# KillingSpark/zstd-rs

Measured on AMD Instinct MI355X. Metric: decompressed_GB_per_s, higher is better.
Workload: dtype u8

## Files before the change

### zstd-rs_amd/csrc/zg_dev.h

```cpp
#pragma once
#include <stdint.h>
#include "zg_types.h"

#if defined(__HIPCC__)
#include <hip/hip_runtime.h>
#define ZG_HD __host__ __device__ __forceinline__
#else
#define ZG_HD static inline __attribute__((always_inline))
#endif

static constexpr uint32_t ZG_LL_BASE[36] = {0, 1, 2, 3, 4, 5, 6, 7, 8, 9, 10, 11, 12, 13, 14, 15, 16, 18, 20, 22, 24, 28, 32, 40,
                                            48, 64, 128, 256, 512, 1024, 2048, 4096, 8192, 16384, 32768, 65536};
static constexpr uint8_t ZG_LL_BITS[36] = {0, 0, 0, 0, 0, 0, 0, 0, 0, 0, 0, 0, 0, 0, 0, 0, 1, 1, 1, 1, 2, 2, 3, 3,
                                           4, 6, 7, 8, 9, 10, 11, 12, 13, 14, 15, 16};
static constexpr uint32_t ZG_ML_BASE[53] = {3, 4, 5, 6, 7, 8, 9, 10, 11, 12, 13, 14, 15, 16, 17, 18, 19, 20, 21, 22, 23, 24, 25, 26, 27, 28, 29,
                                            30, 31, 32, 33, 34, 35, 37, 39, 41, 43, 47, 51, 59, 67, 83, 99, 131, 259, 515, 1027, 2051, 4099,
                                            8195, 16387, 32771, 65539};
static constexpr uint8_t ZG_ML_BITS[53] = {0, 0, 0, 0, 0, 0, 0, 0, 0, 0, 0, 0, 0, 0, 0, 0, 0, 0, 0, 0, 0, 0, 0, 0, 0, 0, 0,
                                           0, 0, 0, 0, 0, 1, 1, 1, 1, 2, 2, 3, 3, 4, 4, 5, 7, 8, 9, 10, 11, 12, 13, 14, 15, 16};
static constexpr int16_t ZG_LL_DEFAULT[36] = {4, 3, 2, 2, 2, 2, 2, 2, 2, 2, 2, 2, 2, 1, 1, 1, 2, 2, 2, 2, 2, 2, 2, 2, 2, 3, 2, 1, 1, 1, 1, 1, -1, -1, -1, -1};
static constexpr int16_t ZG_ML_DEFAULT[53] = {1, 4, 3, 2, 2, 2, 2, 2, 2, 1, 1, 1, 1, 1, 1, 1, 1, 1, 1, 1, 1, 1, 1, 1, 1, 1, 1, 1, 1, 1, 1, 1,
                                              1, 1, 1, 1, 1, 1, 1, 1, 1, 1, 1, 1, 1, 1, -1, -1, -1, -1, -1, -1, -1};
static constexpr int16_t ZG_OF_DEFAULT[29] = {1, 1, 1, 1, 1, 1, 2, 2, 2, 1, 1, 1, 1, 1, 1, 1, 1, 1, 1, 1, 1, 1, 1, 1, -1, -1, -1, -1, -1};

// ... 115 lines not shown
        pos = (pos + step) & (size - 1);
        if (++guard > size) return ZG_INTERNAL;
      }
    }
  }
  if (placed != neg) return ZG_INTERNAL;
  for (uint32_t i = 0; i < neg; i++) {
    unsigned s = out[i];
    uint32_t p = (uint32_t)probs[s], k = counter[s]++;
    unsigned hb = zg_hbit(p);
    uint32_t slices = ((1u << (hb - 1)) == p) ? p : (1u << hb);
    uint32_t dbl = slices - p, single = p - dbl, width = size / slices;
    uint32_t nb = zg_hbit(width) - 1, bl;
    if (k < dbl) { bl = single * width + k * width * 2; nb += 1; }
    else bl = (k - dbl) * width;
    out[i] = zg_fse_pack(kind, bl, nb, s);
  }
  for (uint32_t i = neg; i < size; i++) out[i] = zg_fse_pack(kind, 0, (uint32_t)acc_log, out[i]);
  return ZG_OK;
}

ZG_HD int zg_huf_read_weights(const uint8_t* src, uint32_t len, uint8_t* weights, int* nweights, uint32_t* bytes_used, uint32_t* fse_tab,
                              int16_t* probs, uint16_t* counter) {
  if (len == 0) return ZG_HUF_TABLE;
  uint32_t header = src[0];
  uint32_t bits_read = 8;
  if (header < 128) {
    const uint8_t* fs = src + 1;
    uint32_t flen = len - 1;
    if (header > flen) return ZG_HUF_TABLE;
    int np, al;
    uint32_t used;
    int st = zg_fse_read_probs(fs, flen, 6, 255, probs, &np, &al, &used);
    if (st) return ZG_HUF_TABLE;
    st = zg_fse_build(probs, np, al, ZG_KIND_HUFW, fse_tab, counter);
    if (st) return st == ZG_INTERNAL ? st : ZG_HUF_TABLE;
    if (used > header) return ZG_HUF_TABLE;
    uint32_t clen = header - used;
    const uint8_t* cs = fs + used;
    bits_read += (used + clen) * 8;
    if (clen == 0) return ZG_HUF_TABLE;
    uint32_t lastb = cs[clen - 1];
    if (lastb == 0) return ZG_HUF_TABLE;
    int32_t P = (int32_t)(clen - 1) * 8 + (int32_t)(zg_hbit(lastb) - 1);
    uint32_t e1, e2;
    P -= al; e1 = fse_tab[zg_bits_at_z(cs, P, (unsigned)al)];
    P -= al; e2 = fse_tab[zg_bits_at_z(cs, P, (unsigned)al)];
    int n = 0;
    for (;;) {
      weights[n++] = (uint8_t)ZG_FSEW_SYM(e1);
      { unsigned nb = ZG_FSE_NB(e1); P -= nb; e1 = fse_tab[ZG_FSE_BL(e1) + zg_bits_at_z(cs, P, nb)]; }
      if (P <= -1) { weights[n++] = (uint8_t)ZG_FSEW_SYM(e2); break; }
      weights[n++] = (uint8_t)ZG_FSEW_SYM(e2);
      { unsigned nb = ZG_FSE_NB(e2); P -= nb; e2 = fse_tab[ZG_FSE_BL(e2) + zg_bits_at_z(cs, P, nb)]; }
      if (P <= -1) { weights[n++] = (uint8_t)ZG_FSEW_SYM(e1); break; }
      if (n > 255) return ZG_HUF_TABLE;
    }
    *nweights = n;
  } else {
    uint32_t n = header - 127, need = (n + 1) / 2;
    if (len - 1 < need) return ZG_HUF_TABLE;
    for (uint32_t i = 0; i < n; i++) {
      uint8_t b = src[1 + i / 2];
      weights[i] = (i & 1) ? (b & 0xF) : (b >> 4);
      bits_read += 4;
    }
    *nweights = (int)n;
  }
  *bytes_used = (bits_read + 7) >> 3;
  return ZG_OK;
}

ZG_HD int zg_huf_build(const uint8_t* weights, int nweights, uint16_t* out, int* max_bits_out) {
  uint32_t weight_sum = 0;
  for (int i = 0; i < nweights; i++) {
    unsigned w = weights[i];
    if (w > 11) return ZG_HUF_TABLE;
    weight_sum += w ? (1u << (w - 1)) : 0u;
  }
  if (weight_sum == 0) return ZG_HUF_TABLE;
  unsigned max_bits = zg_hbit(weight_sum);
  uint32_t left = (1u << max_bits) - weight_sum;
  if (left & (left - 1)) return ZG_HUF_TABLE;
  unsigned last_weight = zg_hbit(left);
  if (max_bits > 11) return ZG_HUF_TABLE;
  *max_bits_out = (int)max_bits;
  uint32_t rank_count[13];
  for (int i = 0; i < 13; i++) rank_count[i] = 0;
  for (int s = 0; s <= nweights; s++) {
    unsigned w = s < nweights ? weights[s] : last_weight;
    unsigned b = w ? max_bits + 1 - w : 0;
    rank_count[b]++;
  }
  uint32_t rank_idx[13];
  rank_idx[max_bits] = 0;
  for (unsigned b = max_bits; b >= 1; b--) rank_idx[b - 1] = rank_idx[b] + rank_count[b] * (1u << (max_bits - b));
  uint32_t size = 1u << max_bits;
  if (rank_idx[0] != size) return ZG_INTERNAL;
  for (int s = 0; s <= nweights; s++) {
    unsigned w = s < nweights ? weights[s] : last_weight;
    if (!w) continue;
    unsigned b = max_bits + 1 - w;
    uint32_t base = rank_idx[b], n = 1u << (max_bits - b);
    rank_idx[b] += n;
    uint16_t e = ZG_HUF_PACK((unsigned)(s & 255), b);
    for (uint32_t i = 0; i < n; i++) out[base + i] = e;
  }
  return ZG_OK;
}

#define ZG_OFF_HUGE 0x3FFFFFFFu
#define ZG_SYM_TAG(v) ((v) >> 30)
#define ZG_SYM_K(v) ((v) & 0x3FFFFFFFu)
ZG_HD uint32_t zg_sym_dec(uint32_t v) {
  const uint32_t c = v ? v - 1 : 0u;
  return ZG_SYM_TAG(v) ? v + 1 : c;
}
ZG_HD uint32_t zg_sym_resolve(uint32_t v, const uint32_t* h) {
  uint32_t t = ZG_SYM_TAG(v);
  if (!t) return v;
  const uint32_t x = t == 1 ? h[0] : t == 2 ? h[1] : h[2], k = ZG_SYM_K(v);
  return x > k ? x - k : 0;
}
ZG_HD uint32_t zg_hist_step(uint32_t of, uint32_t ll, uint32_t& h0, uint32_t& h1, uint32_t& h2) {
  const bool isnew = of > 3u;
  const uint32_t c = ll ? of : of + 1u;
  const uint32_t rep = c == 1u ? h0 : c == 2u ? h1 : c == 3u ? h2 : zg_sym_dec(h0);
  const uint32_t actual = isnew ? of - 3u : rep;
  const bool rot = isnew || c >= 3u;
  const bool moved = rot || c == 2u;
  h2 = rot ? h1 : h2;
  h1 = moved ? h0 : h1;
  h0 = actual;
  return actual;
}
struct ZgHistMap { uint32_t s[3]; };
ZG_HD ZgHistMap zg_map_identity() { return {{1u << 30, 2u << 30, 3u << 30}}; }
ZG_HD uint32_t zg_map_apply(const ZgHistMap& A, uint32_t v) {
  const uint32_t t = ZG_SYM_TAG(v);
  if (!t) return v;
  const uint32_t a = t == 1 ? A.s[0] : t == 2 ? A.s[1] : A.s[2], k = ZG_SYM_K(v);
  if (ZG_SYM_TAG(a)) {
    uint32_t kk = ZG_SYM_K(a) + k;
    if (kk > 0x3FFFFFFFu) kk = 0x3FFFFFFFu;
    return (a & 0xC0000000u) | kk;
  }
  return a > k ? a - k : 0;
}
ZG_HD ZgHistMap zg_map_compose(const ZgHistMap& A, const ZgHistMap& B) {
  ZgHistMap r;
  r.s[0] = zg_map_apply(A, B.s[0]); r.s[1] = zg_map_apply(A, B.s[1]); r.s[2] = zg_map_apply(A, B.s[2]);
  return r;
}
```

### zstd-rs_amd/csrc/zg_kernels.hip

```cpp
#include <stdlib.h>
#include "zg_kernels.h"
#include "zg_dev.h"
#include "zg_xxh64_dev.h"
#include "zg_scatter.h"

#define ZG_SEQ_G 16
#define ZG_LZ_T 256

typedef uint32_t zg_v4u __attribute__((ext_vector_type(4)));
typedef __attribute__((address_space(1))) zg_v4u zg_gv4u;
typedef uint32_t zg_v2u __attribute__((ext_vector_type(2)));
typedef __attribute__((address_space(1))) zg_v2u zg_gv2u;
typedef uint32_t zg_v3u __attribute__((ext_vector_type(3)));
typedef __attribute__((address_space(1))) zg_v3u zg_gv3u;
__device__ __forceinline__ uint32_t zg_ld32_fun(const uint8_t* p) {
  const uint64_t a = (uint64_t)p;
  const zg_v2u v = *(const zg_gv2u*)(a & ~3ull);
  return __builtin_amdgcn_alignbit(v.y, v.x, ((uint32_t)a & 3u) * 8u);
}

__device__ __forceinline__ void zg_set_status(uint32_t* status, uint32_t b, int st) {
  if (st) atomicCAS(&status[b], 0u, (uint32_t)st);
}
__device__ __forceinline__ uint32_t zg_sweep_window(const ZgBatchDev& d, const ZgFrame& fr) {
// ... 622 lines not shown
    if (!s_ok[g]) {
      const uint32_t bo = d.aux[b].seq_bits_off;
      const bool nopad = bo <= blk.src_len && (blk.src_len == bo || d.src[blk.src_off + blk.src_len - 1u] == 0);
      if (owner && !mover) zg_set_status(d.status, b, nopad ? ZG_SEQ_EXTRA_PADDING : ZG_FSE_UNINIT);
      act = false;
    } else {
      const uint32_t bits_off = d.aux[b].seq_bits_off;
      if (bits_off > blk.src_len) { if (owner && !mover) zg_set_status(d.status, b, ZG_INTERNAL); act = false; }
      else {
        const uint8_t* bs = d.src + blk.src_off + bits_off;
        const uint32_t bs_len = blk.src_len - bits_off;
        nseq = blk.nseq;
        const uint32_t lastb = bs_len ? bs[bs_len - 1] : 0;
        if (bs_len == 0 || lastb == 0) { if (owner && !mover) zg_set_status(d.status, b, ZG_SEQ_EXTRA_PADDING); act = false; }
        else {
          P = (int32_t)(bs_len - 1) * 8 + (int32_t)(zg_hbit(lastb) - 1);
          bsA = (uint64_t)bs;
          rbits = (int32_t)((uint32_t)(bsA & (ZG_SEQ_RING - 1)) * 8u);
          floorA = (bsA & ~15ull) - 16;
          dstp = (uint64_t)(d.raw_arena + blk.seq_base);
          have = true;
        }
      }
    }
  }
  {
    uint64_t top = 0, want = 0;
    if (act) {
      top = (bsA + (uint64_t)(P >> 3) + 8 + 15) & ~15ull;
      const uint64_t p0 = bsA + (uint64_t)(P >> 3);
      want = p0 > ZG_SEQ_MARGIN + 16 ? (p0 - ZG_SEQ_MARGIN - 16) & ~15ull : 0;
      if (want < floorA) want = floorA;
      lo = want;
    }
    if (owner && !mover) { s_fetch_hi[g] = act ? top : 0; s_fetch_lo[g] = act ? want : 0; }
    __syncthreads();
    for (uint32_t j = t; j < ZG_SEQ_G * ZG_SEQ_PRO; j += 128) {
      const uint32_t gg = j / ZG_SEQ_PRO, k = j % ZG_SEQ_PRO;
      const uint64_t hi = s_fetch_hi[gg], addr = hi - 16ull * (k + 1);
      if (hi && addr >= s_fetch_lo[gg] && addr < hi) { const zg_v4u v = *(const zg_gv4u*)addr; zg_ring_put(s_ring[gg], addr, v); }
    }
    __syncthreads();
  }
  ZgSeqChain c = {0, 0, 0, 0, 0, 0, 0, 0, 0};
  if (act) {
    const uint32_t ll_log = s_log[g][0], of_log = s_log[g][1], ml_log = s_log[g][2];
    const uint32_t lg = role == 0u ? of_log : role == 1u ? ml_log : role == 2u ? ll_log : 0u;
    const int32_t q = P - (int32_t)(role == 2u ? ll_log : role == 0u ? ll_log + of_log : ll_log + of_log + ml_log);
    c.st = (q >= 0 && role != 3u) ? zg_ring_bits(store, q + rbits, lg) : 0u;
    c.e = ZG_SEQ_LD16(tab, c.st); c.s = PK ? 0u : ZG_SEQ_LD8(xtab, c.st);
    P -= (int32_t)(ll_log + of_log + ml_log);
    if (owner && !mover) d.seq_out[b].pad = (uint32_t)P;
    left = nseq;
  }
  c.pr = P + rbits;
#ifdef ZG_PROFILE_SEQ
  unsigned long long tcs[3] = {0, 0, 0}, tl_ = clock64();
#define ZG_QTICK(i) { const unsigned long long n_ = clock64(); tcs[i] += n_ - tl_; tl_ = n_; }
#else
#define ZG_QTICK(i)
#endif
  if (!mover) {
    if (act) zg_seq_window(c, store4);
    for (uint32_t par = 0;; par ^= 1u) {
      uint16_t* const out_base = (uint16_t*)&s_out[par][g][0] + role;
      uint32_t cnt = 0;
      if (act && left > ZG_SEQ_CH) {
#pragma unroll
        for (int k = 0; k < ZG_SEQ_CH; k++) zg_seq_step<true, PK>(c, tab, xtab, store4, out_base + 4 * k, rbits, act, left, cnt, to2, to1);
        cnt = ZG_SEQ_CH; left -= ZG_SEQ_CH;
        if (c.pr < rbits) act = false;
      } else if (act) {
#pragma unroll
        for (int k = 0; k < ZG_SEQ_CH; k++) zg_seq_step<false, PK>(c, tab, xtab, store4, out_base, rbits, act, left, cnt, to2, to1);
      }
      P = c.pr - rbits;
      const bool more = __any(act);
      if (owner) { s_pos[par][g] = P; s_cnt[par][g] = cnt | (act ? 256u : 0u); }
      if (t == 0) s_more[par] = more ? 1u : 0u;
      ZG_QTICK(0)
      __syncthreads();
      ZG_QTICK(1)
      if (!more) break;
    }
    if (have && owner) {
      if (left != 0) status = ZG_SEQ_NOT_ENOUGH_BYTES;
      else if (P > 0) status = ZG_SEQ_EXTRA_BITS;
      zg_set_status(d.status, b, status);
    }
  } else {
    zg_v4u piece[ZG_SEQ_PREG];
    uint64_t piece_addr[ZG_SEQ_PREG];
    bool piece_ok[ZG_SEQ_PREG];
#pragma unroll
    for (int pi = 0; pi < ZG_SEQ_PREG; pi++) { piece[pi] = zg_v4u{0, 0, 0, 0}; piece_addr[pi] = 0; piece_ok[pi] = false; }
    for (uint32_t par = 0;; par ^= 1u) {
      __syncthreads();
      const uint32_t cw = s_cnt[par][g], cnt = cw & 255u;
      const bool live = have && (cw >> 8) != 0u;
      const int32_t pos = s_pos[par][g];
      const bool more = s_more[par] != 0u;
      zg_v2u rec[(ZG_SEQ_CH + 3) / 4];
#pragma unroll
      for (int i = 0; i < (ZG_SEQ_CH + 3) / 4; i++) rec[i] = *(const zg_v2u*)&s_out[par][g][role + 4u * (uint32_t)i];
#pragma unroll
      for (int pi = 0; pi < ZG_SEQ_PREG; pi++) if (piece_ok[pi]) zg_ring_put(store, piece_addr[pi], piece[pi]);
      {
        uint64_t hi = 0, want = 0;
        if (live) {
          const uint64_t p0 = bsA + (uint64_t)(pos >> 3);
          want = p0 > ZG_SEQ_MARGIN ? (p0 - ZG_SEQ_MARGIN) & ~15ull : 0;
          if (want < floorA) want = floorA;
          if (want < lo) { hi = lo; lo = want; }
        }
#pragma unroll
        for (int pi = 0; pi < ZG_SEQ_PREG; pi++) {
          const uint64_t addr = hi - 16ull * (role + 4u * (uint32_t)pi + 1u);
          piece_ok[pi] = hi && addr >= want && addr < hi;
          if (piece_ok[pi]) { piece[pi] = *(const zg_gv4u*)addr; piece_addr[pi] = addr; }
        }
      }
#pragma unroll
      for (int i = 0; i < (ZG_SEQ_CH + 3) / 4; i++) {
        const uint32_t k = role + 4u * (uint32_t)i;
        if (k < cnt) ((__attribute__((address_space(1))) uint32_t*)dstp)[k] = ZG_RAW_PACK(rec[i].x & 0xFFu, (rec[i].x >> 16) & 0x1FFu, rec[i].y & 0x1FFu);
      }
      dstp += (uint64_t)cnt * 4u;
      if (!more) break;
    }
  }
#ifdef ZG_PROFILE_SEQ
  if (t == 0 && d.dbg) { atomicAdd(&d.dbg[16], tcs[0]); atomicAdd(&d.dbg[17], tcs[1]); atomicAdd(&d.dbg[18], 1ull); }
#endif
#undef ZG_QTICK
}

#define ZG_SP_T 256
#define ZG_SP_S 8
template <int S> __device__ __forceinline__ void zg_map_scan_step(ZgHistMap& m, uint32_t lane) {
  ZgHistMap pm;
  pm.s[0] = zx_scan_src<S>(m.s[0], 1u << 30); pm.s[1] = zx_scan_src<S>(m.s[1], 2u << 30); pm.s[2] = zx_scan_src<S>(m.s[2], 3u << 30);
  if (zx_scan_takes<S>(lane)) m = zg_map_compose(pm, m);
}
__device__ __forceinline__ ZgHistMap zg_map_scan_incl(ZgHistMap m, uint32_t lane) {
  zg_map_scan_step<0>(m, lane); zg_map_scan_step<1>(m, lane); zg_map_scan_step<2>(m, lane); zg_map_scan_step<3>(m, lane);
  zg_map_scan_step<4>(m, lane); zg_map_scan_step<5>(m, lane);
  return m;
}
__device__ __forceinline__ ZgHistMap zg_map_shr1(const ZgHistMap& m) {
  ZgHistMap r;
  r.s[0] = zx_shr1(m.s[0], 1u << 30); r.s[1] = zx_shr1(m.s[1], 2u << 30); r.s[2] = zx_shr1(m.s[2], 3u << 30);
  return r;
}
__global__ void __launch_bounds__(ZG_SP_T, 4) zg_k_seqpost(ZgBatchDev d) {
  __shared__ ZgHistMap s_wm[ZG_SP_T / 64];
  __shared__ uint32_t s_wl[ZG_SP_T / 64], s_wo[ZG_SP_T / 64], s_wx[ZG_SP_T / 64];
  __shared__ uint32_t s_err;
  __shared__ uint32_t s_llb[36], s_mlb[53];
  __shared__ uint16_t s_t[ZG_FSE_SLOT_U32];
  __shared__ uint32_t s_tr[ZG_SP_T / 64][64 * 25];
  const uint32_t t = threadIdx.x, lane = t & 63, wv = t >> 6;
  const uint32_t b = d.seq_blocks[blockIdx.x];
  if (d.status[b]) return;
  const ZgBlock blk = d.blocks[b];
  {
    const int32_t sl[3] = {blk.ll_slot, blk.ml_slot, blk.of_slot};
    const uint32_t offs[4] = {ZG_FSE_LL_OFF, ZG_FSE_ML_OFF, ZG_FSE_OF_OFF, ZG_FSE_SLOT_U32};
#pragma unroll
    for (int k = 0; k < 3; k++) {
      const uint32_t* g_t = d.fse_arena + (uint64_t)sl[k] * ZG_FSE_SLOT_U32;
      for (uint32_t i = offs[k] + t; i < offs[k + 1]; i += ZG_SP_T) { const uint32_t v = g_t[i]; s_t[i] = (uint16_t)((ZG_FSE_SYM(v) << 4) | ZG_FSE_NB(v)); }
    }
  }
  const uint32_t nseq = blk.nseq, regen = blk.regen_size;
  const uint32_t wlim = zg_sweep_window(d, d.frames[blk.frame]);
  const uint8_t* bs = d.src + blk.src_off + d.aux[b].seq_bits_off;
  const uint32_t* raw = d.raw_arena + blk.seq_base;
  ZgSeq* out = d.seq_arena + blk.seq_base;
  if (t == 0) s_err = 0xFFFFFFFFu;
  if (t < 36) s_llb[t] = ZG_LL_BASE[t] | ((uint32_t)ZG_LL_BITS[t] << 24);
  if (t < 53) s_mlb[t] = ZG_ML_BASE[t] | ((uint32_t)ZG_ML_BITS[t] << 24);
  ZgHistMap carry = zg_map_identity();
  uint32_t lit_carry = 0, out_carry = 0;
  uint32_t pos_carry = d.seq_out[b].pad;
  uint32_t err_i0 = 0;
  __syncthreads();
  for (uint32_t i0 = 0; i0 < nseq; i0 += ZG_SP_T * ZG_SP_S) {
    const uint32_t ib = i0 + t * ZG_SP_S;
    const uint32_t n = ib < nseq ? (nseq - ib < ZG_SP_S ? nseq - ib : ZG_SP_S) : 0u;
    uint32_t r[ZG_SP_S];
    if (n == ZG_SP_S) {
#pragma unroll
      for (int j = 0; j < ZG_SP_S; j += 4) {
        const zg_v4u v = *(const zg_gv4u*)(raw + ib + j);
        r[j] = v.x; r[j + 1] = v.y; r[j + 2] = v.z; r[j + 3] = v.w;
      }
    } else {
#pragma unroll
      for (int j = 0; j < ZG_SP_S; j++) r[j] = (uint32_t)j < n ? raw[ib + j] : 0u;
    }
    uint32_t codes[ZG_SP_S];
    uint32_t P[ZG_SP_S];
    {
      uint32_t tx = 0;
#pragma unroll
      for (int j = 0; j < ZG_SP_S; j++) {
        const uint32_t e_of = s_t[ZG_FSE_OF_OFF + ZG_RAW_OF(r[j])], e_ml = s_t[ZG_FSE_ML_OFF + ZG_RAW_ML(r[j])], e_ll = s_t[ZG_FSE_LL_OFF + ZG_RAW_LL(r[j])];
        const uint32_t of_code = (e_of >> 4) & 31u, ml_code = e_ml >> 4, ll_code = e_ll >> 4;
        const uint32_t vl = s_llb[ll_code < 36 ? ll_code : 0], vm = s_mlb[ml_code < 53 ? ml_code : 0];
        const uint32_t upd = ib + (uint32_t)j + 1u == nseq ? 0u : (e_of & 15u) + (e_ml & 15u) + (e_ll & 15u);
        const bool have = (uint32_t)j < n;
        codes[j] = have ? of_code | (ml_code << 8) | (ll_code << 16) : 0u;
        P[j] = tx;
        tx += have ? of_code + (vl >> 24) + (vm >> 24) + upd : 0u;
      }
      const uint32_t sx = zx_scan_incl_add(tx);
      if (lane == 63) s_wx[wv] = sx;
      __syncthreads();
      uint32_t before = sx - tx, all = 0;
#pragma unroll
      for (uint32_t w = 0; w < ZG_SP_T / 64; w++) { const uint32_t wx = s_wx[w]; if (w < wv) before += wx; all += wx; }
#pragma unroll
      for (int j = 0; j < ZG_SP_S; j++) P[j] = pos_carry - before - P[j];
      pos_carry -= all;
    }
    uint32_t ll[ZG_SP_S], ml[ZG_SP_S], of[ZG_SP_S];
#pragma unroll
    for (int j = 0; j < ZG_SP_S; j++) {
      const uint32_t of_code = codes[j] & 255u, ml_code = (codes[j] >> 8) & 255u, ll_code = codes[j] >> 16;
      const uint32_t vl = s_llb[ll_code < 36 ? ll_code : 0], vm = s_mlb[ml_code < 53 ? ml_code : 0];
      const uint32_t xb_ll = vl >> 24, xb_ml = vm >> 24;
      const uint32_t q_ll = P[j] - of_code - xb_ml - xb_ll;
      const uint64_t pa = (uint64_t)(bs + (q_ll >> 3));
      const zg_v3u wv = *(const zg_gv3u*)(pa & ~3ull);
      const uint32_t sh = ((uint32_t)pa & 3u) * 8u + (q_ll & 7u);
      const uint32_t lo = __builtin_amdgcn_alignbit(wv.y, wv.x, sh), hi = __builtin_amdgcn_alignbit(wv.z, wv.y, sh);
      const uint32_t ll_add = __builtin_amdgcn_ubfe(lo, 0u, xb_ll);
      const uint32_t ml_add = __builtin_amdgcn_ubfe(__builtin_amdgcn_alignbit(hi, lo, xb_ll), 0u, xb_ml);
      const uint32_t so = xb_ll + xb_ml;
      const uint32_t ov = so >= 32u ? hi : __builtin_amdgcn_alignbit(hi, lo, so);
      const bool have = (uint32_t)j < n;
      ll[j] = have ? (vl & 0xFFFFFFu) + ll_add : 0u;
      ml[j] = have ? (vm & 0xFFFFFFu) + ml_add : 0u;
      of[j] = have ? __builtin_amdgcn_ubfe(ov, 0u, of_code) + (1u << of_code) : 0u;
    }
    uint32_t h0 = 1u << 30, h1 = 2u << 30, h2 = 3u << 30, tl = 0, to = 0, act[ZG_SP_S];
    bool far = false;
#pragma unroll
    for (int j = 0; j < ZG_SP_S; j++) {
      act[j] = 1;
      if (of[j]) {
        const bool tb = of[j] > 3u && of[j] - 3u >= (1u << 30);
        far = far || tb || (of[j] > 3u && of[j] - 3u > wlim);
        act[j] = zg_hist_step(tb ? ZG_OFF_HUGE + 3u : of[j], ll[j], h0, h1, h2);
      }
      tl += ll[j]; to += ll[j] + ml[j];
    }
    const uint32_t sl = zx_scan_incl_add(tl), so = zx_scan_incl_add(to);
    const ZgHistMap sc = zg_map_scan_incl(ZgHistMap{{h0, h1, h2}}, lane);
    if (lane == 63) { s_wm[wv] = sc; s_wl[wv] = sl; s_wo[wv] = so; }
    const ZgHistMap ex = zg_map_shr1(sc);
    __syncthreads();
    ZgHistMap pre = carry, tot = carry;
    uint32_t pl = lit_carry, po = out_carry, totl = lit_carry, toto = out_carry;
#pragma unroll
    for (uint32_t w = 0; w < ZG_SP_T / 64; w++) {
      const ZgHistMap wm = s_wm[w];
      const uint32_t wl = s_wl[w], wo = s_wo[w];
      if (w == wv) pre = tot;
      if (w < wv) { pl += wl; po += wo; }
      tot = zg_map_compose(tot, wm); totl += wl; toto += wo;
    }
    pre = zg_map_compose(pre, ex);
    uint32_t lit_pos = pl + sl - tl, out_pos = po + so - to;
    {
      const bool full = __all(n == ZG_SP_S);
      uint32_t* row = &s_tr[wv][lane * 25u];
      uint32_t bad = 0xFFFFFFFFu;
#pragma unroll
      for (int j = 0; j < ZG_SP_S; j++) {
        if ((uint32_t)j < n) {
          const uint32_t actual = zg_map_apply(pre, act[j]);
          uint32_t e = ZG_OK;
          if ((uint64_t)out_pos + ll[j] + ml[j] >= (1ull << 31)) e = ZG_UNSUPPORTED;
          if ((uint64_t)lit_pos + ll[j] > regen) e = ZG_EXE_NOT_ENOUGH_LITERALS;
          if (actual == 0) e = ZG_EXE_ZERO_OFFSET;
          if (e && bad == 0xFFFFFFFFu) bad = ((t * ZG_SP_S + (uint32_t)j) << 8) | e;
          const uint32_t mdst = out_pos + ll[j];
          const uint32_t w1 = ZG_SEQ_W1(mdst, ml[j]), w2 = ZG_SEQ_W2(lit_pos, ml[j]);
          if (full) { row[3 * j] = actual; row[3 * j + 1] = w1; row[3 * j + 2] = w2; }
          else {
            __attribute__((address_space(1))) uint32_t* qo = (__attribute__((address_space(1))) uint32_t*)(out + ib + j);
            qo[0] = actual; qo[1] = w1; qo[2] = w2;
          }
          lit_pos += ll[j]; out_pos += ll[j] + ml[j];
        }
      }
      if (bad != 0xFFFFFFFFu) atomicMin(&s_err, bad);
      if (full) {
        zg_wave_publish();
        __attribute__((address_space(1))) uint32_t* wo = (__attribute__((address_space(1))) uint32_t*)(out + (ib - lane * ZG_SP_S));
#pragma unroll
        for (int q0 = 0; q0 < ZG_SP_S * 3 * 64 / 4; q0 += 64) {
          const uint32_t m = 4u * ((uint32_t)q0 + lane);
          const uint32_t* src4 = &s_tr[wv][(m / 24u) * 25u + m % 24u];
          const zg_v4u v = {src4[0], src4[1], src4[2], src4[3]};
          *(__attribute__((address_space(1))) zg_v4u*)(wo + m) = v;
        }
      }
    }
    if (far) d.totals[3] = 1u;
    carry = tot; lit_carry = totl; out_carry = toto;
    __syncthreads();
    if (s_err != 0xFFFFFFFFu) { err_i0 = i0; break; }
  }
  if (t == 0) {
    ZgBlockSeqOut so;
    so.sum_ll = lit_carry; so.sum_ml = out_carry - lit_carry;
    so.hist_end[0] = carry.s[0]; so.hist_end[1] = carry.s[1]; so.hist_end[2] = carry.s[2];
    so.pad = s_err != 0xFFFFFFFFu ? err_i0 + (s_err >> 8) + 1u : 0u;
    d.seq_out[b] = so;
    if (s_err != 0xFFFFFFFFu) zg_set_status(d.status, b, (int)(s_err & 0xFFu));
  }
}

#include "zg_seqsize.h"
__global__ void __launch_bounds__(ZG_SZ_T) zg_k_seqsize(ZgBatchDev d) {
  __shared__ ZgSeqSizeLds s_l;
  zg_seqsize_block(d, d.seq_blocks[blockIdx.x], s_l);
}

template <int ZG_SCAN_T, int ZG_SCAN_I>
__global__ void __launch_bounds__(ZG_SCAN_T) zg_k_scan(ZgBatchDev d) {
  __shared__ uint64_t s_size[ZG_SCAN_T / 64];
  __shared__ ZgHistMap s_map[ZG_SCAN_T / 64];
  __shared__ uint32_t s_bad;
  __shared__ uint32_t s_badst;
  __shared__ uint32_t s_slow;
  const uint32_t f = blockIdx.x, t = threadIdx.x;
  const ZgFrame fr = d.frames[f];
  uint64_t carry_size = 0;
  ZgHistMap carry_map = zg_map_identity();
  uint32_t good = fr.nblocks, bad_status = 0;
  __shared__ unsigned long long s_counted;
  uint64_t my_counted = 0;
  if (t == 0) { s_slow = 0; s_counted = 0; }
  constexpr uint32_t CH = ZG_SCAN_T * ZG_SCAN_I;
  for (uint32_t c0 = 0; c0 < fr.nblocks; c0 += CH) {
    uint64_t size[ZG_SCAN_I];
    ZgHistMap m[ZG_SCAN_I];
    uint32_t st[ZG_SCAN_I];
    bool comp[ZG_SCAN_I];
    if (t == 0) { s_bad = 0xFFFFFFFFu; s_badst = 0; }
    __syncthreads();
    uint32_t f_host[ZG_SCAN_I], f_stat[ZG_SCAN_I], f_regen[ZG_SCAN_I], f_nseq[ZG_SCAN_I], f_bt[ZG_SCAN_I];
    ZgBlockSeqOut f_so[ZG_SCAN_I];
#pragma unroll
    for (int j = 0; j < ZG_SCAN_I; j++) {
      const uint32_t i = c0 + t * ZG_SCAN_I + (uint32_t)j;
      const uint32_t b = fr.first_block + (i < fr.nblocks ? i : fr.nblocks - 1u);
      const ZgBlock* blk = &d.blocks[b];
      f_host[j] = blk->host_status; f_regen[j] = blk->regen_size; f_nseq[j] = blk->nseq; f_bt[j] = blk->btype;
      f_stat[j] = d.status[b];
      f_so[j] = d.seq_out[b];
    }
#pragma unroll
    for (int j = 0; j < ZG_SCAN_I; j++) {
      const uint32_t i = c0 + t * ZG_SCAN_I + (uint32_t)j;
      size[j] = 0; m[j] = zg_map_identity(); st[j] = 0; comp[j] = false;
      if (i < fr.nblocks) {
        st[j] = f_host[j] ? f_host[j] : f_stat[j];
        comp[j] = f_bt[j] == ZG_BT_COMPRESSED;
        if (!comp[j] || f_nseq[j] == 0) size[j] = f_regen[j];
        else {
          size[j] = (uint64_t)f_regen[j] + f_so[j].sum_ml;
          if (size[j] > ZG_FLAT_MAX) s_slow = 1;
          m[j].s[0] = f_so[j].hist_end[0]; m[j].s[1] = f_so[j].hist_end[1]; m[j].s[2] = f_so[j].hist_end[2];
        }
        if (st[j]) atomicMin(&s_bad, t * ZG_SCAN_I + (uint32_t)j);
      }
    }
    __syncthreads();
    const uint32_t bad = s_bad;
    uint64_t tsum = 0;
    ZgHistMap tmapl = zg_map_identity();
#pragma unroll
    for (int j = 0; j < ZG_SCAN_I; j++) {
      if (t * ZG_SCAN_I + (uint32_t)j >= bad) { size[j] = 0; m[j] = zg_map_identity(); }
      if (comp[j]) my_counted += size[j];
      tsum += size[j];
      tmapl = zg_map_compose(tmapl, m[j]);
    }
    uint64_t isz = tsum;
    ZgHistMap im = tmapl;
    {
      const uint32_t lane = t & 63;
#pragma unroll
      for (int off = 1; off < 64; off <<= 1) {
        const uint32_t lo = __shfl_up((uint32_t)isz, off, 64), hi = __shfl_up((uint32_t)(isz >> 32), off, 64);
        ZgHistMap pm;
        pm.s[0] = __shfl_up(im.s[0], off, 64); pm.s[1] = __shfl_up(im.s[1], off, 64); pm.s[2] = __shfl_up(im.s[2], off, 64);
        if ((int)lane >= off) { isz += ((uint64_t)hi << 32) | lo; im = zg_map_compose(pm, im); }
      }
      if (lane == 63) { s_size[t >> 6] = isz; s_map[t >> 6] = im; }
    }
    __syncthreads();
    uint64_t wsz = 0, tsz = 0;
    ZgHistMap wmap = zg_map_identity(), tmap = zg_map_identity();
    for (uint32_t w = 0; w < ZG_SCAN_T / 64; w++) {
      if (w < (t >> 6)) { wsz += s_size[w]; wmap = zg_map_compose(wmap, s_map[w]); }
      tsz += s_size[w]; tmap = zg_map_compose(tmap, s_map[w]);
    }
    ZgHistMap prev;
    prev.s[0] = __shfl_up(im.s[0], 1, 64); prev.s[1] = __shfl_up(im.s[1], 1, 64); prev.s[2] = __shfl_up(im.s[2], 1, 64);
    if ((t & 63) == 0) prev = zg_map_identity();
    {
      uint64_t excl = carry_size + wsz + isz - tsum;
      ZgHistMap pre = zg_map_compose(zg_map_compose(carry_map, wmap), prev);
#pragma unroll
      for (int j = 0; j < ZG_SCAN_I; j++) {
        const uint32_t li = t * ZG_SCAN_I + (uint32_t)j, i = c0 + li;
        if (i < fr.nblocks) {
          ZgBlockPos p;
          p.out_base = excl;
          p.hist_init[0] = zg_sym_resolve(pre.s[0], fr.hist_init);
          p.hist_init[1] = zg_sym_resolve(pre.s[1], fr.hist_init);
          p.hist_init[2] = zg_sym_resolve(pre.s[2], fr.hist_init);
          p.active = li < bad ? 1u : 0u;
          d.pos[fr.first_block + i] = p;
          if (li == bad) s_badst = st[j];
        }
        excl += size[j];
        pre = zg_map_compose(pre, m[j]);
      }
    }
    __syncthreads();
    if (bad != 0xFFFFFFFFu) {
      good = c0 + bad;
      bad_status = s_badst;
      carry_size += tsz;
      carry_map = zg_map_compose(carry_map, tmap);
      for (uint32_t j = c0 + CH + t; j < fr.nblocks; j += ZG_SCAN_T) d.pos[fr.first_block + j].active = 0;
      break;
    }
    carry_size += tsz;
    carry_map = zg_map_compose(carry_map, tmap);
    __syncthreads();
  }
  if (my_counted) atomicAdd(&s_counted, (unsigned long long)my_counted);
  __syncthreads();
  if (t == 0) {
    ZgFrameOut fo;
    fo.counted = s_counted;
    fo.out_base = 0; fo.out_size = carry_size; fo.status = bad_status; fo.bad_block = good;
    fo.hist_end[0] = zg_sym_resolve(carry_map.s[0], fr.hist_init);
    fo.hist_end[1] = zg_sym_resolve(carry_map.s[1], fr.hist_init);
    fo.hist_end[2] = zg_sym_resolve(carry_map.s[2], fr.hist_init);
    fo.good_blocks = good;
    fo.fast = (s_slow || (d.flags & 1u)) ? 0u : 1u;
    fo.err_packed = 0xFFFFFFFFu;
    fo.og_base = 0;
    if (d.nframes == 1u) {
// ... 687 lines not shown
```

Measured before the change: 112.0.

## Precompute packed FSE entries and specialize seqpost for full tiles

Replaces the 16-bit symbol table plus separate base tables with one 32-bit packed shared table holding base, extra bits, state bits and their sum. This removes the second lookup and the per-sequence arithmetic. Adds compile-time full-tile variants that drop per-element bounds checks. It also moves the last-sequence state-bit correction out of the hot loop, aligns the bitstream base once, and runs the detailed error checks only when a cheap summary test flags a problem. The costs are a larger shared table, extra staging work per block and more code size.

```diff
diff --git a/zstd-rs_amd/csrc/zg_dev.h b/zstd-rs_amd/csrc/zg_dev.h
--- a/zstd-rs_amd/csrc/zg_dev.h
+++ b/zstd-rs_amd/csrc/zg_dev.h
@@ -291,3 +291,23 @@
   r.s[0] = zg_map_apply(A, B.s[0]); r.s[1] = zg_map_apply(A, B.s[1]); r.s[2] = zg_map_apply(A, B.s[2]);
   return r;
 }
+
+ZG_HD uint32_t zg_spe_make(uint32_t base, uint32_t xb, uint32_t nb) { return base | (xb << 17) | (nb << 22) | ((xb + nb) << 26); }
+ZG_HD uint32_t zg_spe_code(int kind, uint32_t fse) {
+  const uint32_t sym = ZG_FSE_SYM(fse);
+  return kind == ZG_KIND_LL ? (sym < 36u ? sym : 0u) : kind == ZG_KIND_ML ? (sym < 53u ? sym : 0u) : sym & 31u;
+}
+ZG_HD uint32_t zg_spe_pack(int kind, uint32_t fse) {
+  const uint32_t c = zg_spe_code(kind, fse), nb = ZG_FSE_NB(fse);
+  return kind == ZG_KIND_LL ? zg_spe_make(ZG_LL_BASE[c], ZG_LL_BITS[c], nb) : kind == ZG_KIND_ML ? zg_spe_make(ZG_ML_BASE[c], ZG_ML_BITS[c], nb) : zg_spe_make(0u, c, nb);
+}
+ZG_HD uint32_t zg_spe_base(uint32_t e) { return e & 0x1FFFFu; }
+ZG_HD uint32_t zg_spe_xb(uint32_t e) { return (e >> 17) & 31u; }
+ZG_HD uint32_t zg_spe_nb(uint32_t e) { return (e >> 22) & 15u; }
+ZG_HD uint32_t zg_spe_bits(uint32_t e) { return e >> 26; }
+
+ZG_HD bool zg_sp_exec_suspect(uint32_t out_end, uint32_t lit_end, uint32_t regen, uint32_t min_actual) {
+  return out_end >= (1u << 31) || lit_end > regen || min_actual == 0u;
+}
+ZG_HD uint32_t zg_sp_offset_limit(uint32_t wlim) { return (wlim < ZG_OFF_HUGE ? wlim : ZG_OFF_HUGE) + 3u; }
+ZG_HD bool zg_sp_offset_suspect(uint32_t max_of, uint32_t wlim) { return max_of > zg_sp_offset_limit(wlim); }
diff --git a/zstd-rs_amd/csrc/zg_kernels.hip b/zstd-rs_amd/csrc/zg_kernels.hip
--- a/zstd-rs_amd/csrc/zg_kernels.hip
+++ b/zstd-rs_amd/csrc/zg_kernels.hip
@@ -798,42 +798,55 @@
   r.s[0] = zx_shr1(m.s[0], 1u << 30); r.s[1] = zx_shr1(m.s[1], 2u << 30); r.s[2] = zx_shr1(m.s[2], 3u << 30);
   return r;
 }
+struct ZgFormFull { static constexpr bool value = true; };
+struct ZgFormAny { static constexpr bool value = false; };
 __global__ void __launch_bounds__(ZG_SP_T, 4) zg_k_seqpost(ZgBatchDev d) {
   __shared__ ZgHistMap s_wm[ZG_SP_T / 64];
   __shared__ uint32_t s_wl[ZG_SP_T / 64], s_wo[ZG_SP_T / 64], s_wx[ZG_SP_T / 64];
   __shared__ uint32_t s_err;
-  __shared__ uint32_t s_llb[36], s_mlb[53];
-  __shared__ uint16_t s_t[ZG_FSE_SLOT_U32];
+  __shared__ uint32_t s_e[ZG_FSE_SLOT_U32];
   __shared__ uint32_t s_tr[ZG_SP_T / 64][64 * 25];
   const uint32_t t = threadIdx.x, lane = t & 63, wv = t >> 6;
   const uint32_t b = d.seq_blocks[blockIdx.x];
   if (d.status[b]) return;
   const ZgBlock blk = d.blocks[b];
   {
-    const int32_t sl[3] = {blk.ll_slot, blk.ml_slot, blk.of_slot};
-    const uint32_t offs[4] = {ZG_FSE_LL_OFF, ZG_FSE_ML_OFF, ZG_FSE_OF_OFF, ZG_FSE_SLOT_U32};
-#pragma unroll
-    for (int k = 0; k < 3; k++) {
-      const uint32_t* g_t = d.fse_arena + (uint64_t)sl[k] * ZG_FSE_SLOT_U32;
-      for (uint32_t i = offs[k] + t; i < offs[k + 1]; i += ZG_SP_T) { const uint32_t v = g_t[i]; s_t[i] = (uint16_t)((ZG_FSE_SYM(v) << 4) | ZG_FSE_NB(v)); }
+    uint32_t* s_llb = &s_tr[0][0], *s_mlb = &s_tr[0][64];
+    if (t < 36) s_llb[t] = zg_spe_make(ZG_LL_BASE[t], ZG_LL_BITS[t], 0u);
+    if (t >= 64 && t < 64 + 53) s_mlb[t - 64] = zg_spe_make(ZG_ML_BASE[t - 64], ZG_ML_BITS[t - 64], 0u);
+    const uint32_t* g_ll = d.fse_arena + (uint64_t)blk.ll_slot * ZG_FSE_SLOT_U32;
+    const uint32_t* g_ml = d.fse_arena + (uint64_t)blk.ml_slot * ZG_FSE_SLOT_U32;
+    const uint32_t* g_of = d.fse_arena + (uint64_t)blk.of_slot * ZG_FSE_SLOT_U32;
+    static_assert(ZG_FSE_ML_OFF % ZG_SP_T == 0 && ZG_FSE_OF_OFF % ZG_SP_T == 0 && ZG_FSE_SLOT_U32 % ZG_SP_T == 0, "a step of the staging loop stays in one table");
+    uint32_t v[ZG_FSE_SLOT_U32 / ZG_SP_T];
+#pragma unroll
+    for (uint32_t k = 0; k < ZG_FSE_SLOT_U32 / ZG_SP_T; k++)
+      v[k] = (k < ZG_FSE_ML_OFF / ZG_SP_T ? g_ll : k < ZG_FSE_OF_OFF / ZG_SP_T ? g_ml : g_of)[k * ZG_SP_T + t];
+    __syncthreads();
+#pragma unroll
+    for (uint32_t k = 0; k < ZG_FSE_SLOT_U32 / ZG_SP_T; k++) {
+      const uint32_t nb = zg_spe_make(0u, 0u, ZG_FSE_NB(v[k]));
+      s_e[k * ZG_SP_T + t] = k < ZG_FSE_ML_OFF / ZG_SP_T   ? s_llb[zg_spe_code(ZG_KIND_LL, v[k])] + nb
+                             : k < ZG_FSE_OF_OFF / ZG_SP_T ? s_mlb[zg_spe_code(ZG_KIND_ML, v[k])] + nb
+                                                           : zg_spe_pack(ZG_KIND_OF, v[k]);
     }
   }
   const uint32_t nseq = blk.nseq, regen = blk.regen_size;
-  const uint32_t wlim = zg_sweep_window(d, d.frames[blk.frame]);
-  const uint8_t* bs = d.src + blk.src_off + d.aux[b].seq_bits_off;
+  const uint32_t of_lim = zg_sp_offset_limit(zg_sweep_window(d, d.frames[blk.frame]));
+  const uint64_t bsa = (uint64_t)(d.src + blk.src_off + d.aux[b].seq_bits_off);
+  const __attribute__((address_space(1))) uint8_t* bs4 = (const __attribute__((address_space(1))) uint8_t*)(bsa & ~3ull);
   const uint32_t* raw = d.raw_arena + blk.seq_base;
   ZgSeq* out = d.seq_arena + blk.seq_base;
   if (t == 0) s_err = 0xFFFFFFFFu;
-  if (t < 36) s_llb[t] = ZG_LL_BASE[t] | ((uint32_t)ZG_LL_BITS[t] << 24);
-  if (t < 53) s_mlb[t] = ZG_ML_BASE[t] | ((uint32_t)ZG_ML_BITS[t] << 24);
   ZgHistMap carry = zg_map_identity();
   uint32_t lit_carry = 0, out_carry = 0;
-  uint32_t pos_carry = d.seq_out[b].pad;
+  uint32_t pos_carry = d.seq_out[b].pad + ((uint32_t)bsa & 3u) * 8u;
   uint32_t err_i0 = 0;
   __syncthreads();
   for (uint32_t i0 = 0; i0 < nseq; i0 += ZG_SP_T * ZG_SP_S) {
     const uint32_t ib = i0 + t * ZG_SP_S;
     const uint32_t n = ib < nseq ? (nseq - ib < ZG_SP_S ? nseq - ib : ZG_SP_S) : 0u;
+    const bool full = __all(n == ZG_SP_S);
     uint32_t r[ZG_SP_S];
     if (n == ZG_SP_S) {
 #pragma unroll
@@ -845,20 +858,29 @@
 #pragma unroll
       for (int j = 0; j < ZG_SP_S; j++) r[j] = (uint32_t)j < n ? raw[ib + j] : 0u;
     }
-    uint32_t codes[ZG_SP_S];
     uint32_t P[ZG_SP_S];
     {
       uint32_t tx = 0;
-#pragma unroll
-      for (int j = 0; j < ZG_SP_S; j++) {
-        const uint32_t e_of = s_t[ZG_FSE_OF_OFF + ZG_RAW_OF(r[j])], e_ml = s_t[ZG_FSE_ML_OFF + ZG_RAW_ML(r[j])], e_ll = s_t[ZG_FSE_LL_OFF + ZG_RAW_LL(r[j])];
-        const uint32_t of_code = (e_of >> 4) & 31u, ml_code = e_ml >> 4, ll_code = e_ll >> 4;
-        const uint32_t vl = s_llb[ll_code < 36 ? ll_code : 0], vm = s_mlb[ml_code < 53 ? ml_code : 0];
-        const uint32_t upd = ib + (uint32_t)j + 1u == nseq ? 0u : (e_of & 15u) + (e_ml & 15u) + (e_ll & 15u);
-        const bool have = (uint32_t)j < n;
-        codes[j] = have ? of_code | (ml_code << 8) | (ll_code << 16) : 0u;
-        P[j] = tx;
-        tx += have ? of_code + (vl >> 24) + (vm >> 24) + upd : 0u;
+      auto bits = [&](auto form) {
+        constexpr bool FULL = decltype(form)::value;
+#pragma unroll
+        for (int j = 0; j < ZG_SP_S; j++) {
+          const uint32_t e_of = s_e[ZG_FSE_OF_OFF + ZG_RAW_OF(r[j])], e_ml = s_e[ZG_FSE_ML_OFF + ZG_RAW_ML(r[j])], e_ll = s_e[ZG_FSE_LL_OFF + ZG_RAW_LL(r[j])];
+          const bool have = FULL || (uint32_t)j < n;
+          P[j] = tx;
+          tx += have ? zg_spe_bits(e_of) + zg_spe_bits(e_ml) + zg_spe_bits(e_ll) : 0u;
+        }
+      };
+      if (full) bits(ZgFormFull{}); else bits(ZgFormAny{});
+      if (nseq - ib - 1u < ZG_SP_S) {
+        uint32_t upd = 0;
+#pragma unroll
+        for (int j = 0; j < ZG_SP_S; j++) {
+          P[j] -= upd;
+          if (ib + (uint32_t)j + 1u == nseq)
+            upd = zg_spe_nb(s_e[ZG_FSE_OF_OFF + ZG_RAW_OF(r[j])]) + zg_spe_nb(s_e[ZG_FSE_ML_OFF + ZG_RAW_ML(r[j])]) + zg_spe_nb(s_e[ZG_FSE_LL_OFF + ZG_RAW_LL(r[j])]);
+        }
+        tx -= upd;
       }
       const uint32_t sx = zx_scan_incl_add(tx);
       if (lane == 63) s_wx[wv] = sx;
@@ -871,37 +893,37 @@
       pos_carry -= all;
     }
     uint32_t ll[ZG_SP_S], ml[ZG_SP_S], of[ZG_SP_S];
-#pragma unroll
-    for (int j = 0; j < ZG_SP_S; j++) {
-      const uint32_t of_code = codes[j] & 255u, ml_code = (codes[j] >> 8) & 255u, ll_code = codes[j] >> 16;
-      const uint32_t vl = s_llb[ll_code < 36 ? ll_code : 0], vm = s_mlb[ml_code < 53 ? ml_code : 0];
-      const uint32_t xb_ll = vl >> 24, xb_ml = vm >> 24;
-      const uint32_t q_ll = P[j] - of_code - xb_ml - xb_ll;
-      const uint64_t pa = (uint64_t)(bs + (q_ll >> 3));
-      const zg_v3u wv = *(const zg_gv3u*)(pa & ~3ull);
-      const uint32_t sh = ((uint32_t)pa & 3u) * 8u + (q_ll & 7u);
-      const uint32_t lo = __builtin_amdgcn_alignbit(wv.y, wv.x, sh), hi = __builtin_amdgcn_alignbit(wv.z, wv.y, sh);
-      const uint32_t ll_add = __builtin_amdgcn_ubfe(lo, 0u, xb_ll);
-      const uint32_t ml_add = __builtin_amdgcn_ubfe(__builtin_amdgcn_alignbit(hi, lo, xb_ll), 0u, xb_ml);
-      const uint32_t so = xb_ll + xb_ml;
-      const uint32_t ov = so >= 32u ? hi : __builtin_amdgcn_alignbit(hi, lo, so);
-      const bool have = (uint32_t)j < n;
-      ll[j] = have ? (vl & 0xFFFFFFu) + ll_add : 0u;
-      ml[j] = have ? (vm & 0xFFFFFFu) + ml_add : 0u;
-      of[j] = have ? __builtin_amdgcn_ubfe(ov, 0u, of_code) + (1u << of_code) : 0u;
-    }
     uint32_t h0 = 1u << 30, h1 = 2u << 30, h2 = 3u << 30, tl = 0, to = 0, act[ZG_SP_S];
     bool far = false;
-#pragma unroll
-    for (int j = 0; j < ZG_SP_S; j++) {
-      act[j] = 1;
-      if (of[j]) {
-        const bool tb = of[j] > 3u && of[j] - 3u >= (1u << 30);
-        far = far || tb || (of[j] > 3u && of[j] - 3u > wlim);
-        act[j] = zg_hist_step(tb ? ZG_OFF_HUGE + 3u : of[j], ll[j], h0, h1, h2);
-      }
-      tl += ll[j]; to += ll[j] + ml[j];
-    }
+    auto values = [&](auto form) {
+      constexpr bool FULL = decltype(form)::value;
+#pragma unroll
+      for (int j = 0; j < ZG_SP_S; j++) {
+        const bool have = FULL || (uint32_t)j < n;
+        const uint32_t vl = have ? s_e[ZG_FSE_LL_OFF + ZG_RAW_LL(r[j])] : 0u, vm = have ? s_e[ZG_FSE_ML_OFF + ZG_RAW_ML(r[j])] : 0u;
+        const uint32_t of_code = have ? zg_spe_xb(s_e[ZG_FSE_OF_OFF + ZG_RAW_OF(r[j])]) : 0u;
+        const uint32_t xb_ll = zg_spe_xb(vl), xb_ml = zg_spe_xb(vm);
+        const uint32_t q_ll = P[j] - of_code - xb_ml - xb_ll;
+        const zg_v3u wv = *(const zg_gv3u*)(bs4 + ((q_ll >> 5) << 2));
+        const uint32_t sh = q_ll & 31u;
+        const uint32_t lo = __builtin_amdgcn_alignbit(wv.y, wv.x, sh), hi = __builtin_amdgcn_alignbit(wv.z, wv.y, sh);
+        const uint32_t ll_add = __builtin_amdgcn_ubfe(lo, 0u, xb_ll);
+        const uint32_t ml_add = __builtin_amdgcn_ubfe(__builtin_amdgcn_alignbit(hi, lo, xb_ll), 0u, xb_ml);
+        const uint32_t so = xb_ll + xb_ml;
+        const uint32_t ov = so >= 32u ? hi : __builtin_amdgcn_alignbit(hi, lo, so);
+        ll[j] = have ? zg_spe_base(vl) + ll_add : 0u;
+        ml[j] = have ? zg_spe_base(vm) + ml_add : 0u;
+        of[j] = have ? __builtin_amdgcn_ubfe(ov, 0u, of_code) + (1u << of_code) : 0u;
+        far = far || of[j] > of_lim;
+      }
+#pragma unroll
+      for (int j = 0; j < ZG_SP_S; j++) {
+        act[j] = 1;
+        if (FULL || of[j]) act[j] = zg_hist_step(of[j] < ZG_OFF_HUGE + 3u ? of[j] : ZG_OFF_HUGE + 3u, ll[j], h0, h1, h2);
+        tl += ll[j]; to += ll[j] + ml[j];
+      }
+    };
+    if (full) values(ZgFormFull{}); else values(ZgFormAny{});
     const uint32_t sl = zx_scan_incl_add(tl), so = zx_scan_incl_add(to);
     const ZgHistMap sc = zg_map_scan_incl(ZgHistMap{{h0, h1, h2}}, lane);
     if (lane == 63) { s_wm[wv] = sc; s_wl[wv] = sl; s_wo[wv] = so; }
@@ -920,40 +942,54 @@
     pre = zg_map_compose(pre, ex);
     uint32_t lit_pos = pl + sl - tl, out_pos = po + so - to;
     {
-      const bool full = __all(n == ZG_SP_S);
-      uint32_t* row = &s_tr[wv][lane * 25u];
-      uint32_t bad = 0xFFFFFFFFu;
-#pragma unroll
-      for (int j = 0; j < ZG_SP_S; j++) {
-        if ((uint32_t)j < n) {
-          const uint32_t actual = zg_map_apply(pre, act[j]);
-          uint32_t e = ZG_OK;
-          if ((uint64_t)out_pos + ll[j] + ml[j] >= (1ull << 31)) e = ZG_UNSUPPORTED;
-          if ((uint64_t)lit_pos + ll[j] > regen) e = ZG_EXE_NOT_ENOUGH_LITERALS;
-          if (actual == 0) e = ZG_EXE_ZERO_OFFSET;
-          if (e && bad == 0xFFFFFFFFu) bad = ((t * ZG_SP_S + (uint32_t)j) << 8) | e;
-          const uint32_t mdst = out_pos + ll[j];
-          const uint32_t w1 = ZG_SEQ_W1(mdst, ml[j]), w2 = ZG_SEQ_W2(lit_pos, ml[j]);
-          if (full) { row[3 * j] = actual; row[3 * j + 1] = w1; row[3 * j + 2] = w2; }
-          else {
-            __attribute__((address_space(1))) uint32_t* qo = (__attribute__((address_space(1))) uint32_t*)(out + ib + j);
-            qo[0] = actual; qo[1] = w1; qo[2] = w2;
+      auto records = [&](auto form) {
+        constexpr bool FULL = decltype(form)::value;
+        uint32_t* row = &s_tr[wv][lane * 25u];
+        uint32_t least = 0xFFFFFFFFu;
+#pragma unroll
+        for (int j = 0; j < ZG_SP_S; j++) {
+          if (FULL || (uint32_t)j < n) {
+            const uint32_t actual = zg_map_apply(pre, act[j]);
+            least = actual < least ? actual : least;
+            const uint32_t mdst = out_pos + ll[j];
+            const uint32_t w1 = ZG_SEQ_W1(mdst, ml[j]), w2 = ZG_SEQ_W2(lit_pos, ml[j]);
+            if (FULL) { row[3 * j] = actual; row[3 * j + 1] = w1; row[3 * j + 2] = w2; }
+            else {
+              __attribute__((address_space(1))) uint32_t* qo = (__attribute__((address_space(1))) uint32_t*)(out + ib + j);
+              qo[0] = actual; qo[1] = w1; qo[2] = w2;
+            }
+            lit_pos += ll[j]; out_pos += ll[j] + ml[j];
           }
-          lit_pos += ll[j]; out_pos += ll[j] + ml[j];
         }
-      }
-      if (bad != 0xFFFFFFFFu) atomicMin(&s_err, bad);
-      if (full) {
-        zg_wave_publish();
-        __attribute__((address_space(1))) uint32_t* wo = (__attribute__((address_space(1))) uint32_t*)(out + (ib - lane * ZG_SP_S));
-#pragma unroll
-        for (int q0 = 0; q0 < ZG_SP_S * 3 * 64 / 4; q0 += 64) {
-          const uint32_t m = 4u * ((uint32_t)q0 + lane);
-          const uint32_t* src4 = &s_tr[wv][(m / 24u) * 25u + m % 24u];
-          const zg_v4u v = {src4[0], src4[1], src4[2], src4[3]};
-          *(__attribute__((address_space(1))) zg_v4u*)(wo + m) = v;
+        if (zg_sp_exec_suspect(out_pos, lit_pos, regen, least)) {
+          uint32_t lp = lit_pos - tl, op = out_pos - to, bad = 0xFFFFFFFFu;
+#pragma unroll
+          for (int j = 0; j < ZG_SP_S; j++) {
+            if (FULL || (uint32_t)j < n) {
+              const uint32_t actual = zg_map_apply(pre, act[j]);
+              uint32_t e = ZG_OK;
+              if ((uint64_t)op + ll[j] + ml[j] >= (1ull << 31)) e = ZG_UNSUPPORTED;
+              if ((uint64_t)lp + ll[j] > regen) e = ZG_EXE_NOT_ENOUGH_LITERALS;
+              if (actual == 0) e = ZG_EXE_ZERO_OFFSET;
+              if (e && bad == 0xFFFFFFFFu) bad = ((uint32_t)j << 8) | e;
+              lp += ll[j]; op += ll[j] + ml[j];
+            }
+          }
+          if (bad != 0xFFFFFFFFu) atomicMin(&s_err, ((t * ZG_SP_S) << 8) + bad);
         }
-      }
+        if (FULL) {
+          zg_wave_publish();
+          __attribute__((address_space(1))) uint32_t* wo = (__attribute__((address_space(1))) uint32_t*)(out + (ib - lane * ZG_SP_S));
+#pragma unroll
+          for (int q0 = 0; q0 < ZG_SP_S * 3 * 64 / 4; q0 += 64) {
+            const uint32_t m = 4u * ((uint32_t)q0 + lane);
+            const uint32_t* src4 = &s_tr[wv][(m / 24u) * 25u + m % 24u];
+            const zg_v4u v = {src4[0], src4[1], src4[2], src4[3]};
+            *(__attribute__((address_space(1))) zg_v4u*)(wo + m) = v;
+          }
+        }
+      };
+      if (full) records(ZgFormFull{}); else records(ZgFormAny{});
     }
     if (far) d.totals[3] = 1u;
     carry = tot; lit_carry = totl; out_carry = toto;
```

Result: no change. 113.3 (median of 6 runs) (+1.2%).
